# Algolzw/image-restoration-sde

Measured on AMD Instinct MI355X. Metric: restored images/sec at 256x256, 100-step IR-SDE reverse sampler, higher is better.
Workload: dtype f32; 1 GPU; IR-SDE deraining ConditionalUNet nf=64 depth=4, reverse_sde, batch=16/GPU 256x256, T=100 (BASELINE.json configs[1]); compute_dtype=fp32, global_batch=16

## Files before the change

### image_restoration_sde_amd/csrc/engine_api.hip

```cpp
#include "engine.h"
#include <cmath>
#include "../../include/irsde_hip_debug.h"

using namespace irsde;

namespace irsde {
namespace {

thread_local std::string g_last_error;

hipEvent_t get_event(irsde_engine* e, size_t i) {
    while (e->ev_pool.size() <= i) {
        hipEvent_t ev;
        IRSDE_HIP_CHECK(hipEventCreate(&ev));
        e->ev_pool.push_back(ev);
    }
    return e->ev_pool[i];
}

void run_net(Plan* pl, hipStream_t s) {
    for (auto& op : pl->net_ops) op.fn(s);
}

UpdateParams make_update(irsde_engine* e, Plan* pl) {
    UpdateParams u{};
    u.x = pl->xin; u.mu = pl->cin; u.pred = pl->pred;
    const int64_t ps = pl->pred_stride;
    u.sb = (int64_t)pl->Hp * pl->Wp * ps; u.sc = 1; u.sy = (int64_t)pl->Wp * ps; u.sx = ps;
    u.st = pl->own_step ? pl->own_step : e->step; u.ctl = e->ctl;
    u.B = pl->B; u.C = e->cfg.in_nc; u.H = pl->H; u.W = pl->W;
    u.batch0 = pl->b0;
    return u;
}

void one_step(irsde_engine* e, Plan* pl, hipStream_t s) {
    launch_step_begin(e->step, e->film_table, e->film_row, e->film_cur, e->coef_table, s);
    run_net(pl, s);
    launch_sde_update(make_update(e, pl), s);
}

void ensure_sub_streams(irsde_engine* e, int n) {
    if (!e->ev_fork) IRSDE_HIP_CHECK(hipEventCreateWithFlags(&e->ev_fork, hipEventDisableTiming));
    for (int i = 0; i + 1 < n; ++i) {
        if (!e->sub_stream[i]) IRSDE_HIP_CHECK(hipStreamCreateWithFlags(&e->sub_stream[i], hipStreamNonBlocking));
        if (!e->ev_join[i]) IRSDE_HIP_CHECK(hipEventCreateWithFlags(&e->ev_join[i], hipEventDisableTiming));
    }
}
void one_step_part(irsde_engine* e, Plan* pl, hipStream_t s) {
    launch_step_begin(pl->own_step, e->film_table, e->film_row, pl->own_film, e->coef_table, s);
    run_net(pl, s);
    launch_sde_update(make_update(e, pl), s);
}

struct VariantScope {
    explicit VariantScope(int v) { conv_set_variant(v); }
    ~VariantScope() { conv_set_variant(0); }
};

bool code_in(const std::initializer_list<int>& codes, int c) { return std::find(codes.begin(), codes.end(), c) != codes.end(); }
bool debug_conv_code_known(int c) {
    return code_in({0, 1, 2, 3, 4, 5, 12, 13, 22, 23, 33, 34, 35, 36, 37, 42, 43, 44, 45, 46, 47, 55, 56, 62, 63, 204, 260, 261, 262, 263}, c) ||
           code_in({100, 103, 105, 106, 107, 150, 160, 161, 162, 163, 165, 166, 167, 170, 171, 172, 173}, c);
}
bool bench_conv_variant_known(int v) {
    return code_in({0, 3, 5, 6, 7, 50, 60, 61, 62, 63, 64, 65, 66, 67, 70, 71, 72, 73}, v) ||
           code_in({80, 81, 82, 412, 413, 421, 422, 423, 430, 431, 432, 434, 435, 460, 461, 462, 465, 467, 468, 469, 480, 481, 482}, v) ||
           code_in({2001, 2002, 2004, 4650, 4651, 4652, 4653}, v) ||
           (v >= 83 && v <= 82 + 255) ||
           (v >= 472 && v <= 476);
}

void apply_fp16_flag(irsde_engine* e) {
    if (!(e->cfg.flags & IRSDE_FLAG_FP16)) return;
    if (e->cfg.flags & IRSDE_FLAG_BF16_ACT) {
        delete e;
        throw HipError("IRSDE_FLAG_FP16 keeps fp32 activation storage: it cannot be combined with IRSDE_FLAG_BF16_ACT");
    }
    e->cfg.flags |= IRSDE_FLAG_BF16;
}

int guard(const std::function<void()>& f) {
    try {
        f();
        return IRSDE_OK;
    } catch (const HipError& ex) {
        g_last_error = ex.what();
        const std::string m = ex.what();
        if (m.find("weight") != std::string::npos) return IRSDE_ERR_WEIGHT;
        if (m.find(" failed: ") != std::string::npos) return IRSDE_ERR_HIP;
        return IRSDE_ERR_INVALID;
    } catch (const std::exception& ex) {
        g_last_error = ex.what();
        return IRSDE_ERR_INVALID;
    }
}

}
}

extern "C" {

const char* irsde_last_error(void) { return g_last_error.c_str(); }
int irsde_version(void) { return 107; }

int irsde_create(const irsde_config* cfg, irsde_engine** out) {
    return guard([&] {
        if (!cfg || !out) throw HipError("null argument");
        if (cfg->nf % 32 || cfg->nf < 32) throw HipError("nf must be a positive multiple of 32");
        if (cfg->depth < 1 || cfg->depth > 6) throw HipError("depth out of range");
        if (cfg->in_nc < 1 || cfg->in_nc > 4 || cfg->out_nc < 1 || cfg->out_nc > 4)
            throw HipError("in_nc/out_nc must be in 1..4");
        if (cfg->in_nc != cfg->out_nc) throw HipError("sampler needs in_nc == out_nc");
        if ((cfg->nf << cfg->depth) > 2048) throw HipError("nf * 2^depth must be <= 2048");
        if (cfg->flags & IRSDE_FLAG_NAF_STEREO) throw HipError("IRSDE_FLAG_NAF_STEREO: the stereo network is a ConditionalNAFNet (irsde_create_nafnet)");
        if (cfg->flags & IRSDE_FLAG_NAF_UNCOND) throw HipError("IRSDE_FLAG_NAF_UNCOND: irsde_create_nafnet only (the unconditional UNet is IRSDE_FLAG_UNCOND_FULLATTN)");
        auto* e = new irsde_engine();
        e->cfg = *cfg;
        if (cfg->flags & IRSDE_FLAG_BF16_ACT) {
            if (cfg->flags & (IRSDE_FLAG_UNCOND_FULLATTN | IRSDE_FLAG_NAIVE_CONV)) {
                delete e;
// ... 456 lines not shown
int irsde_debug_scam(const float* x, int B, int H, int W, int C, const float* norm_l_g, const float* norm_r_g, const float* l_proj1_w,
                     const float* l_proj1_b, const float* r_proj1_w, const float* r_proj1_b, const float* l_proj2_w, const float* l_proj2_b,
                     const float* r_proj2_w, const float* r_proj2_b, const float* beta, const float* gamma, float* out, void* stream) {
    return guard([&] {
        if (!x || !out || !norm_l_g || !norm_r_g || !l_proj1_w || !l_proj1_b || !r_proj1_w || !r_proj1_b || !l_proj2_w || !l_proj2_b || !r_proj2_w ||
            !r_proj2_b || !beta || !gamma)
            throw HipError("null argument");
        if (B < 1) throw HipError("debug_scam: bad shape");
        scam_check_shape(H, W, C);
        hipStream_t s = reinterpret_cast<hipStream_t>(stream);
        conv_global_init();
        const int Hs = H / 4, Ws = W / 4;
        std::vector<float> wl, bl, wr, br;
        scam_pack_proj(l_proj1_w, l_proj1_b, l_proj2_w, l_proj2_b, C, wl, bl);
        scam_pack_proj(r_proj1_w, r_proj1_b, r_proj2_w, r_proj2_b, C, wr, br);
        std::vector<float*> bufs;
        auto up = [&](const float* h, size_t n) {
            float* d = nullptr;
            IRSDE_HIP_CHECK(hipMalloc(&d, std::max<size_t>(n, 16) * 4));
            bufs.push_back(d);
            if (h) IRSDE_HIP_CHECK(hipMemcpy(d, h, n * 4, hipMemcpyHostToDevice));
            return d;
        };
        try {
            float *dgl = up(norm_l_g, C), *dgr = up(norm_r_g, C), *dbe = up(beta, C), *dga = up(gamma, C);
            float *dwl = up(wl.data(), wl.size()), *dbl = up(bl.data(), bl.size()), *dwr = up(wr.data(), wr.size()), *dbr = up(br.data(), br.size());
            const size_t vsz = (size_t)B * Hs * Ws * 2 * C;
            float *xs2 = up(nullptr, 2 * vsz), *qv = up(nullptr, 2 * vsz), *F = up(nullptr, vsz), *dz = up(nullptr, 256);
            IRSDE_HIP_CHECK(hipMemset(dz, 0, 1024));
            launch_scam_prologue(x, dgl, dgr, xs2, B, H, W, C, s);
            for (int v = 0; v < 2; ++v) {
                ConvParams p;
                p.in0 = xs2 + v * vsz; p.C0 = 2 * C; p.pix0 = 2 * C;
                p.Hin = Hs; p.Win = Ws;
                p.w = v ? dwr : dwl; p.Cout = 2 * C; p.KH = p.KW = 1; p.stride = 1;
                p.B = B; p.Ho = Hs; p.Wo = Ws;
                p.out = qv + v * vsz; p.out_stride = 2 * C;
                p.bias = v ? dbr : dbl;
                p.zeros = dz;
                launch_conv(p, s);
            }
            launch_scam_core(qv, F, B, H, W, C, s);
            launch_scam_epilogue(x, F, dbe, dga, out, B, H, W, C, s);
            IRSDE_HIP_CHECK(hipStreamSynchronize(s));
        } catch (...) {
            (void)hipStreamSynchronize(s);
            for (float* p : bufs) (void)hipFree(p);
            throw;
        }
        for (float* p : bufs) (void)hipFree(p);
    });
}

int irsde_debug_conv(const float* in0, int C0, const float* in1, int C1, int B, int Hin, int Win, int in_shift,
                     const float* w_oihw, int Cout, int KH, int KW, int stride, int pad, const float* bias,
                     const float* film, int film_bstride, int silu, const float* res, float* out, int naive,
                     int splits, void* stream) {
    return guard([&] {
        if (!in0 || !w_oihw || !out) throw HipError("null argument");
        if (!debug_conv_code_known(naive)) throw HipError("debug_conv: unknown selector code " + std::to_string(naive));
        hipStream_t s = reinterpret_cast<hipStream_t>(stream);
        conv_global_init();
        const int Cin = C0 + C1;
        std::vector<float> pk((size_t)Cout * KH * KW * Cin);
        for (int o = 0; o < Cout; ++o)
            for (int i = 0; i < Cin; ++i)
                for (int ky = 0; ky < KH; ++ky)
                    for (int kx = 0; kx < KW; ++kx)
                        pk[(((size_t)o * KH + ky) * KW + kx) * Cin + i] = w_oihw[(((size_t)o * Cin + i) * KH + ky) * KW + kx];
        float *dw = nullptr, *db = nullptr, *dp = nullptr;
        IRSDE_HIP_CHECK(hipMalloc(&dw, pk.size() * 4));
        IRSDE_HIP_CHECK(hipMemcpy(dw, pk.data(), pk.size() * 4, hipMemcpyHostToDevice));
        if (bias) {
            IRSDE_HIP_CHECK(hipMalloc(&db, Cout * 4));
            IRSDE_HIP_CHECK(hipMemcpy(db, bias, Cout * 4, hipMemcpyHostToDevice));
        }
        ConvParams p;
        p.in0 = in0; p.C0 = C0; p.pix0 = C0; p.in1 = in1; p.C1 = C1; p.pix1 = C1;
        p.Hin = Hin; p.Win = Win; p.in_shift = in_shift;
        p.w = dw; p.Cout = Cout; p.KH = KH; p.KW = KW; p.stride = stride; p.pad_y = pad; p.pad_x = pad;
        p.B = B;
        p.Ho = ((Hin << in_shift) + 2 * pad - KH) / stride + 1;
        p.Wo = ((Win << in_shift) + 2 * pad - KW) / stride + 1;
        p.out = out; p.out_stride = Cout; p.bias = db; p.film = film; p.film_bstride = film_bstride; p.silu = silu;
        p.res = res; p.res_stride = Cout;
        float* dz = nullptr;
        IRSDE_HIP_CHECK(hipMalloc(&dz, 1024));
        IRSDE_HIP_CHECK(hipMemset(dz, 0, 1024));
        p.zeros = dz;
        const int wino_tile = (naive == 2 || naive == 12 || naive == 22) ? 2 : (naive == 3 || naive == 13 || naive == 23) ? 4 : 0;
        if (splits > 1 && naive != 1 && !wino_tile) {
            p.splits = splits;
            IRSDE_HIP_CHECK(hipMalloc(&dp, (size_t)splits * B * p.Ho * p.Wo * Cout * 4));
            p.partial = dp;
        }
        if (naive == 44 || naive == 45) {
            const bool f16 = naive == 44;
            if (!wino_shape_ok(p, 4) || Cin % 32) throw HipError("debug_conv: shape not eligible for the pair GEMM");
            std::vector<float> U((size_t)36 * Cout * Cin);
            wino_transform_weights(pk.data(), Cout, Cin, U.data(), 4);
            float mx = 0.f;
            for (float v : U) mx = std::max(mx, std::fabs(v));
            const float us = f16 && mx > 0.f ? std::exp2(std::floor(std::log2(512.0f / mx))) : 1.f;
            const long long T = (long long)B * (p.Ho / 4) * (p.Wo / 4);
            float *dU = nullptr, *dM = nullptr;
            unsigned short *dUp = nullptr, *dVp = nullptr;
            IRSDE_HIP_CHECK(hipMalloc(&dU, U.size() * 4));
            IRSDE_HIP_CHECK(hipMemcpy(dU, U.data(), U.size() * 4, hipMemcpyHostToDevice));
            IRSDE_HIP_CHECK(hipMalloc(&dUp, U.size() * 4));
            IRSDE_HIP_CHECK(hipMalloc(&dVp, (size_t)36 * T * Cin * 4));
            IRSDE_HIP_CHECK(hipMalloc(&dM, (size_t)36 * T * Cout * 4));
            launch_split_pairs(dU, dUp, (size_t)36 * Cout, Cin, s, f16, us);
            const WinoSplitPlan sp = make_wino_pairs(p, dUp, dVp, dM, f16, us);
            launch_wino_input(sp.in, s);
            launch_gemm_split_pairs(sp.gemm, 36, s, 0, f16);
            launch_wino_output(sp.out, s);
            IRSDE_HIP_CHECK(hipStreamSynchronize(s));
            (void)hipFree(dU); (void)hipFree(dUp); (void)hipFree(dVp); (void)hipFree(dM);
        } else if (naive == 42 || naive == 43) {
            const int npl = naive - 40;
            if (!wino_shape_ok(p, 4)) throw HipError("debug_conv: shape not eligible for Winograd");
            std::vector<float> U((size_t)36 * Cout * Cin);
            wino_transform_weights(pk.data(), Cout, Cin, U.data(), 4);
            const long long T = (long long)B * (p.Ho / 4) * (p.Wo / 4);
            float *dU = nullptr, *dM = nullptr;
            unsigned short *dUs = nullptr, *dVs = nullptr;
            IRSDE_HIP_CHECK(hipMalloc(&dU, U.size() * 4));
            IRSDE_HIP_CHECK(hipMemcpy(dU, U.data(), U.size() * 4, hipMemcpyHostToDevice));
            IRSDE_HIP_CHECK(hipMalloc(&dUs, U.size() * 2 * npl));
            IRSDE_HIP_CHECK(hipMalloc(&dVs, (size_t)36 * T * Cin * 2 * npl));
            IRSDE_HIP_CHECK(hipMalloc(&dM, (size_t)36 * T * Cout * 4));
            launch_split_planes(dU, dUs, U.size(), U.size(), npl, s);
            const WinoSplitPlan sp = make_wino_split(p, dUs, dVs, dM, npl);
            launch_wino_input(sp.in, s);
            launch_gemm_split(sp.gemm, npl, 36, s);
            launch_wino_output(sp.out, s);
            IRSDE_HIP_CHECK(hipStreamSynchronize(s));
            (void)hipFree(dU); (void)hipFree(dUs); (void)hipFree(dVs); (void)hipFree(dM);
// ... 409 lines not shown
                IRSDE_HIP_CHECK(hipMalloc(&dM, (size_t)36 * T * Cout * 4));
                wp = make_wino(p, dU, dV, dM, 4);
                if (variant == 421) launch_wino_input(wp.in, s);
            }
            if (split_v) {
                if (!wino_shape_ok(p, 4)) throw HipError("bench_conv: shape not eligible for Winograd F(4x4,3x3)");
                const int npl = variant % 10;
                const long long T = (long long)B * (p.Ho / 4) * (p.Wo / 4);
                const size_t nu = (size_t)36 * Cout * Cin;
                IRSDE_HIP_CHECK(hipMalloc(&dUs, nu * 2 * npl));
                IRSDE_HIP_CHECK(hipMalloc(&dVs, (size_t)36 * T * Cin * 2 * npl));
                IRSDE_HIP_CHECK(hipMalloc(&dM, (size_t)36 * T * Cout * 4));
                launch_split_planes(dU, dUs, nu, nu, npl, s);
                sp = make_wino_split(p, dUs, dVs, dM, npl);
                launch_wino_input(sp.in, s);
            }
        }
        if (variant == 82) {
            IRSDE_HIP_CHECK(hipMalloc(&dU, (size_t)36 * nw / 9 * 4));
            launch_fill_random(dU, (size_t)36 * nw / 9, 5, 1.0f / sqrtf((float)(9 * Cin)), s);
            const int nb = wino_fused_num_blocks(p);
            unsigned long long* dd = nullptr;
            IRSDE_HIP_CHECK(hipMalloc(&dd, (size_t)nb * 128 * 8));
            launch_wino_fused(p, dU, s);
            IRSDE_HIP_CHECK(hipMemsetAsync(dd, 0, (size_t)nb * 128 * 8, s));
            launch_wino_fused(p, dU, s, dd);
            IRSDE_HIP_CHECK(hipStreamSynchronize(s));
            std::vector<unsigned long long> hd((size_t)nb * 128);
            IRSDE_HIP_CHECK(hipMemcpy(hd.data(), dd, hd.size() * 8, hipMemcpyDeviceToHost));
            double ph[2][4] = {{0, 0, 0, 0}, {0, 0, 0, 0}};
            unsigned long long rt_min = ~0ull, rt_max = 0;
            for (int bi = 0; bi < nb; ++bi)
                for (int w = 0; w < 8; ++w) {
                    const unsigned long long* t = &hd[((size_t)bi * 8 + w) * 16];
                    for (int k = 0; k < 4; ++k) ph[w >= 4][k] += (double)(t[k + 1] - t[k]) / ((double)nb * 4);
                    rt_min = std::min(rt_min, t[7]);
                    rt_max = std::max(rt_max, t[7]);
                }
            printf("wino_fused timeline B=%d %dx%d Cin=%d Cout=%d: %d blocks, block starts span %.1f us\n", B, p.Ho, p.Wo, Cin, Cout, nb,
                   (double)(rt_max - rt_min) / 100.0);
            printf("  MFMA waves     (shader cycles): start->V[0] ready %.0f | K loop %.0f | acc->LDS+barrier %.0f | epilogue %.0f\n", ph[0][0],
                   ph[0][1], ph[0][2], ph[0][3]);
            printf("  producer waves (shader cycles): start->chunk 0 done %.0f | K loop rest %.0f | wait MFMA+acc %.0f | epilogue %.0f\n",
                   ph[1][0], ph[1][1], ph[1][2], ph[1][3]);
            fflush(stdout);
            (void)hipFree(dd);
            (void)hipFree(dU);
            dU = nullptr;
            *ms_out = 0.0;
            (void)hipFree(din); (void)hipFree(dw); (void)hipFree(dout); (void)hipFree(dres); (void)hipFree(dfilm);
            (void)hipStreamDestroy(s);
            return;
        }
        if (variant == 465 || (variant >= 4650 && variant <= 4653)) {
            if (!wino_fused64t_eligible(p)) throw HipError("bench_conv: shape not eligible for the two-tile-group fused Winograd kernel");
            const int nbp = 256;
            unsigned long long* dd = nullptr;
            IRSDE_HIP_CHECK(hipMalloc(&dd, (size_t)nbp * 64 * 8));
            launch_wino_fused64t(p, dU, s, 0);
            IRSDE_HIP_CHECK(hipMemsetAsync(dd, 0, (size_t)nbp * 64 * 8, s));
            wino_fused64t_set_debug(dd);
            launch_wino_fused64t(p, dU, s, variant == 465 ? 5 : 12 + (variant - 4650));
            IRSDE_HIP_CHECK(hipStreamSynchronize(s));
            wino_fused64t_set_debug(nullptr);
            std::vector<unsigned long long> hd((size_t)nbp * 64);
            IRSDE_HIP_CHECK(hipMemcpy(hd.data(), dd, hd.size() * 8, hipMemcpyDeviceToHost));
            double a5[8] = {0, 0, 0, 0, 0, 0, 0, 0};
            int nwv = 0;
            for (int bi = 0; bi < nbp; ++bi)
                for (int w = 0; w < 8; ++w) {
                    const unsigned long long* t = &hd[((size_t)bi * 8 + w) * 8];
                    if (!t[3]) continue;
                    for (int k = 0; k < 8; ++k) a5[k] += (double)t[k];
                    nwv++;
                }
            const int nst = Cin / 16;
            const double items = a5[4] / std::max(nwv, 1), chunks = items * nst;
            printf("wino4_fused64t stamps B=%d %dx%d Cin=%d Cout=%d: %.1f items x %d chunks of 16 channels per block; shader cycles per wave (mean over %d waves)\n", B, p.Ho, p.Wo, Cin,
                   Cout, items, nst, nwv);
            printf("  kernel %.0f = K loops incl. transform slices %.0f (%.0f per chunk; MFMA floor per SIMD 9216) + chunk barrier waits %.0f (%.0f per chunk) + epilogue, exchange, first-chunk transform %.0f (%.0f per item)\n",
                   a5[3] / nwv, a5[0] / nwv, a5[0] / nwv / chunks, a5[1] / nwv, a5[1] / nwv / chunks, (a5[2] + a5[5] + a5[6] + a5[7]) / nwv, (a5[2] + a5[5] + a5[6] + a5[7]) / nwv / items);
            printf("  per item: first stage + exchange writes + ring %.0f | exchange barriers + reads %.0f | second stage, stores, gathers %.0f | zero, first-chunk transform, barrier %.0f\n",
                   a5[5] / nwv / items, a5[6] / nwv / items, a5[7] / nwv / items, a5[2] / nwv / items);
            fflush(stdout);
            (void)hipFree(dd);
            (void)hipFree(dU);
            dU = nullptr;
            *ms_out = 0.0;
            (void)hipFree(din); (void)hipFree(dw); (void)hipFree(dout); (void)hipFree(dres); (void)hipFree(dfilm);
            (void)hipStreamDestroy(s);
            return;
        }
        if (variant == 435 || (variant >= 2001 && variant <= 2004)) {
            const int stamp_variant = variant == 2001 ? 28 : variant == 2002 ? 29 : 25;
            const int nbp = 256;
            unsigned long long* dd = nullptr;
            IRSDE_HIP_CHECK(hipMalloc(&dd, (size_t)nbp * 64 * 8));
            launch_wino_fused64(p, dU, s, 20);
            IRSDE_HIP_CHECK(hipMemsetAsync(dd, 0, (size_t)nbp * 64 * 8, s));
            wino_fused64_set_debug(dd);
            launch_wino_fused64(p, dU, s, stamp_variant);
            IRSDE_HIP_CHECK(hipStreamSynchronize(s));
            wino_fused64_set_debug(nullptr);
            std::vector<unsigned long long> hd((size_t)nbp * 64);
            IRSDE_HIP_CHECK(hipMemcpy(hd.data(), dd, hd.size() * 8, hipMemcpyDeviceToHost));
            double acc[2][5] = {{0, 0, 0, 0, 0}, {0, 0, 0, 0, 0}};
            int nw[2] = {0, 0};
// ... 265 lines not shown
```

### image_restoration_sde_amd/csrc/wino_fused_t.hip

```cpp
#include "common.h"
#include "wino_fused_shared.h"
#include <mutex>

namespace irsde {

namespace {

constexpr int WT_NT = 512;
constexpr int WT_KC = 16;
constexpr int WT_PS = 256;
constexpr int WT_ZS = 2 * WT_PS;
constexpr int WT_VBUF = 36 * WT_ZS;
constexpr int WT_XCH_BYTES = 8 * 12 * 64 * 16;
constexpr int WT_RES_BYTES = 8 * 8 * 1024;
constexpr int WT_LDS_BYTES = 160 * 1024;
static_assert(WT_XCH_BYTES + WT_RES_BYTES <= WT_LDS_BYTES && 2 * WT_VBUF * 4 <= WT_LDS_BYTES, "LDS budget");
constexpr unsigned WT_ROW_OOB = 0x80000000u;
constexpr unsigned WT_COL_OOB = 0x40000000u;

__device__ __forceinline__ void swap32x6(float& a0, float& b0, float& a1, float& b1, float& a2, float& b2, float& a3, float& b3, float& a4, float& b4,
                                         float& a5, float& b5) {
    asm volatile(
        "s_nop 1\n\tv_permlane32_swap_b32 %0, %1\n\tv_permlane32_swap_b32 %2, %3\n\tv_permlane32_swap_b32 %4, %5\n\t"
        "v_permlane32_swap_b32 %6, %7\n\tv_permlane32_swap_b32 %8, %9\n\tv_permlane32_swap_b32 %10, %11"
        : "+v"(a0), "+v"(b0), "+v"(a1), "+v"(b1), "+v"(a2), "+v"(b2), "+v"(a3), "+v"(b3), "+v"(a4), "+v"(b4), "+v"(a5), "+v"(b5));
}

template <int H>
__device__ __forceinline__ void wt_stage1(const floatx4 (&acc)[18][2], floatx4 (&keep)[12], float* xs) {
#pragma unroll
    for (int tg = 0; tg < 2; ++tg) {
        floatx4 u[4][3];
#pragma unroll
        for (int sc = 0; sc < 3; ++sc) {
            const floatx4 m0 = acc[sc][tg], m1 = acc[3 + sc][tg], m2 = acc[6 + sc][tg], m3 = acc[9 + sc][tg], m4 = acc[12 + sc][tg], m5 = acc[15 + sc][tg];
            const floatx4 s12 = m1 + m2, d12 = m1 - m2, s34 = m3 + m4, d34 = m3 - m4;
            u[0][sc] = m0 + s12 + s34;
            u[1][sc] = d12 + 2.0f * d34;
            u[2][sc] = s12 + 4.0f * s34;
            u[3][sc] = d12 + 8.0f * d34 + m5;
        }
#pragma unroll
        for (int i = 0; i < 4; ++i) {
            const floatx4 t0 = H == 0 ? u[i][0] : u[i][0] + u[i][1];
            const floatx4 t1 = H == 0 ? u[i][1] + u[i][2] : u[i][0] - u[i][1];
            const floatx4 t2 = H == 0 ? u[i][1] - u[i][2] : u[i][2];
            if (tg == H) {
                keep[3 * i] = t0; keep[3 * i + 1] = t1; keep[3 * i + 2] = t2;
            } else {
                *reinterpret_cast<floatx4*>(xs + (3 * i) * 256) = t0;
                *reinterpret_cast<floatx4*>(xs + (3 * i + 1) * 256) = t1;
                *reinterpret_cast<floatx4*>(xs + (3 * i + 2) * 256) = t2;
            }
        }
    }
}

template <int H, int HALF, bool RES, bool SILU>
__device__ __forceinline__ void wt_finish_rows(const ConvParams& p, const floatx4 (&keep)[12], const floatx4 (&recv)[12], const floatx4 (&rv)[2][4],
                                               const unsigned lane_off_out, const __amdgpu_buffer_rsrc_t rs_out, const floatx4 bias, const floatx4 fsc,
                                               const floatx4 fsh) {
    constexpr int AUX = 2;
    const int orow = p.Wo * p.out_stride * 4, opix = p.out_stride * 4;
#pragma unroll
    for (int ii = 0; ii < 2; ++ii) {
        const int i = 2 * HALF + ii;
        const floatx4 u0 = H == 0 ? keep[3 * i] : recv[3 * i], s12 = H == 0 ? keep[3 * i + 1] : recv[3 * i + 1], d12 = H == 0 ? keep[3 * i + 2] : recv[3 * i + 2];
        const floatx4 s34 = H == 0 ? recv[3 * i] : keep[3 * i], d34 = H == 0 ? recv[3 * i + 1] : keep[3 * i + 1], u5 = H == 0 ? recv[3 * i + 2] : keep[3 * i + 2];
        floatx4 y[4];
        y[0] = u0 + s12 + s34;
        y[1] = d12 + 2.0f * d34;
        y[2] = s12 + 4.0f * s34;
        y[3] = d12 + 8.0f * d34 + u5;
#pragma unroll
        for (int j = 0; j < 4; ++j) {
            floatx4 v = (y[j] + bias) * fsc + fsh;
            if constexpr (SILU) {
                v.x = silu_w(v.x); v.y = silu_w(v.y); v.z = silu_w(v.z); v.w = silu_w(v.w);
            }
            if constexpr (RES) v = v + rv[ii][j];
            __builtin_amdgcn_raw_buffer_store_b128(__builtin_bit_cast(__attribute__((__vector_size__(4 * sizeof(unsigned)))) unsigned, v), rs_out,
                                                   (int)(lane_off_out + (unsigned)(i * orow + j * opix)), 0, AUX);
        }
    }
}

constexpr int WT_NR = 6;

template <bool NOWT, bool NOPATCH, int EPI, bool STAMP = false, int DBG = 0>
__global__ __launch_bounds__(WT_NT, 2) void wino4_fused64t_kernel(const ConvParams p, const float* __restrict__ Uf, const int GX, const int GY, const int NB,
                                                                   const unsigned in0_bytes, const unsigned in1_bytes, const unsigned uf_bytes,
                                                                   const unsigned out_bytes, const unsigned res_bytes, const int xcd_nb, const int total,
                                                                   unsigned long long* __restrict__ dbg) {
    static_assert(18 % WT_NR == 0, "the ring must divide the 18 weight units of a chunk");
    constexpr bool RES = (EPI & 2) != 0, SILU = (EPI & 1) != 0;
    unsigned long long st_a = 0, st_b = 0, st_c = 0, st_n = 0, st_t0 = 0, st_t = 0, st_e1 = 0, st_e2 = 0, st_e3 = 0;
    if constexpr (STAMP) st_t0 = st_t = __builtin_amdgcn_s_memtime();
#define WT_STAMP(ACC)                                                     \
    if constexpr (STAMP) {                                                \
        const unsigned long long now_ = __builtin_amdgcn_s_memtime();     \
        ACC += now_ - st_t;                                               \
        st_t = now_;                                                      \
    }
    extern __shared__ __attribute__((aligned(16))) float smem[];
    const int tid = threadIdx.x;
    const int lane = tid & 63;
    const int wave = __builtin_amdgcn_readfirstlane(tid >> 6);
    const int cb = wave & 3, h = wave >> 2;
    const int TH = p.Ho >> 2, TW = p.Wo >> 2;
    const int Ctot = p.C0 + p.C1;
    const int nch = Ctot / WT_KC;
    const int nblocks = gridDim.x;
    const int l15 = lane & 15, g = lane >> 4;
    const __amdgpu_buffer_rsrc_t rsrc_u = __builtin_amdgcn_make_buffer_rsrc(const_cast<float*>(Uf), 0, NOWT ? 0u : uf_bytes, 0x00020000);
    const __amdgpu_buffer_rsrc_t rs_out = __builtin_amdgcn_make_buffer_rsrc(p.out, 0, out_bytes, 0x00020000);
    const __amdgpu_buffer_rsrc_t rs_res = __builtin_amdgcn_make_buffer_rsrc(const_cast<float*>(p.res ? p.res : p.out), 0, p.res ? res_bytes : 0u, 0x00020000);
    floatx4 acc[18][2];
    const floatx4 kZero4 = {0.f, 0.f, 0.f, 0.f};
    const int uv_lane = lane * 16;
    const int zstride = NB * nch * 4096;
    int v = blockIdx.x;
    W6Item it = w6_item(v, total, NB, GX, GY, xcd_nb);
    int ubase = it.nblk * nch * 4096 + cb * 1024 + 3 * h * zstride;
    auto unit_rel = [&](const int zl) { return ((zl / 3) * 6 + zl % 3) * zstride; };
    floatx4 ring[WT_NR];
    const int v_lane = g * 64 + (((l15 ^ (2 * g)) & 15) * 4);
    const __amdgpu_buffer_rsrc_t rsrc0 = __builtin_amdgcn_make_buffer_rsrc(const_cast<float*>(p.in0), 0, NOPATCH ? 0u : in0_bytes, 0x00020000);
    const __amdgpu_buffer_rsrc_t rsrc1 =
        __builtin_amdgcn_make_buffer_rsrc(const_cast<float*>(p.in1 ? p.in1 : p.in0), 0, (p.in1 && !NOPATCH) ? in1_bytes : 0u, 0x00020000);
    const int hh = lane >> 5, tl = (lane >> 3) & 3, cp = lane & 7;
    const int ptile = 4 * (wave & 3) + tl, ptg = wave >> 2;
    const int kg = cp >> 1;
    const int vw_base = hh * (18 * WT_ZS) + ptg * WT_PS + kg * 64 + (((ptile ^ (2 * kg)) & 15) * 4) + 2 * (cp & 1);
    const int Hv = p.Hin << p.in_shift, Wv = p.Win << p.in_shift;
    floatx2 raw[18];
    unsigned rowoff[6], coloff[3];
#pragma unroll
// ... 92 lines not shown
                    if (u < 3) { WT_GATHER_ROW(2 * u) WT_GATHER_ROW(2 * u + 1) }                                             \
                    if (u == 2) { WT_ADVANCE() WT_SETUP() }                                                                  \
                }                                                                                                            \
                if constexpr (!(DBG & 1)) { if (u >= TC && u < TC + 3) WT_COLPASS(u - TC) }                                  \
                if constexpr (!(DBG & 4)) { if (u == TC + 3) WT_SWAPS() }                                                    \
                if constexpr (!(DBG & 2)) { if (u >= TC + 4 && u < TC + 7) WT_ROWPASS_WRITE(u - TC - 4, wbuf) }              \
                if constexpr (GA && !(DBG & 8)) {                                                                            \
                    if constexpr (FIRST) {                                                                                   \
                        if (u >= 16) { WT_GATHER_ROW(3 * (u - 16)) WT_GATHER_ROW(3 * (u - 16) + 1) WT_GATHER_ROW(3 * (u - 16) + 2) } \
                    } else {                                                                                                 \
                        if (u >= 13 && u < 16) { WT_GATHER_ROW(2 * (u - 13)) WT_GATHER_ROW(2 * (u - 13) + 1) }               \
                    }                                                                                                        \
                }                                                                                                            \
                __builtin_amdgcn_sched_barrier(0);                                                                           \
            }                                                                                                                \
            if (!(LAST) || u + WT_NR < 18) {    \
                const int K = u + WT_NR;                                                                                     \
                const int off = K < 18 ? cur_off + unit_rel(K) : cur_off + 4096 + unit_rel(K - 18);                          \
                ring[u % WT_NR] = __builtin_bit_cast(floatx4, __builtin_amdgcn_raw_buffer_load_b128(rsrc_u, uv_lane, off, 0)); \
            }                                                                                                                \
            __builtin_amdgcn_sched_barrier(0);                                                                               \
        }                                                                                                                    \
        if constexpr (GA) WT_ADVANCE()                                                                                       \
        WT_STAMP(st_a)                                                                                                       \
        __syncthreads();                                                                                                     \
        WT_STAMP(st_b)                                                                                                       \
    }

    WT_SETUP()
#pragma unroll
    for (int i = 0; i < 6; ++i) WT_GATHER_ROW(i)
    WT_ADVANCE()
#pragma unroll
    for (int i = 0; i < WT_NR; ++i)
        ring[i] = __builtin_bit_cast(floatx4, __builtin_amdgcn_raw_buffer_load_b128(rsrc_u, uv_lane, ubase + unit_rel(i), 0));
#pragma unroll
    for (int j = 0; j < 3; ++j) WT_COLPASS(j)
    WT_SWAPS()
#pragma unroll
    for (int r = 0; r < 3; ++r) WT_ROWPASS_WRITE(r, 0)
    WT_SETUP()
    __syncthreads();
    WT_STAMP(st_c)
    while (v < total) {
        const int nv = v + nblocks;
        nit = w6_item(nv < total ? nv : v, total, NB, GX, GY, xcd_nb);
        const int nubase = nit.nblk * nch * 4096 + cb * 1024 + 3 * h * zstride;
        WT_CHUNK(0, true, true, false, true)
        for (int c = 1; c < nch - 2; ++c) WT_CHUNK(c, true, true, false, false)
        WT_CHUNK(nch - 2, true, false, false, false)
        WT_CHUNK(nch - 1, false, false, true, false)
        {
            const int n = it.nblk * 64 + cb * 16 + 4 * g;
            const int tyy = it.gy * 4 + (l15 >> 2), txx = it.gx * 8 + h * 4 + (l15 & 3);
            const bool ok = tyy < TH && txx < TW;
            const unsigned pix = (unsigned)((it.b * p.Ho + 4 * tyy) * p.Wo + 4 * txx);
            unsigned off_out = ok ? (pix * (unsigned)p.out_stride + (unsigned)n) * 4u : WF_OOB;
            unsigned off_res = ok ? (pix * (unsigned)p.res_stride + (unsigned)n) * 4u : WF_OOB;
            if constexpr ((DBG & 128) != 0) {
                const int tx4 = it.gx * 8 + h * 4 + cb;
                const unsigned pixc = (unsigned)((it.b * p.Ho + 4 * tyy) * p.Wo + 4 * tx4);
                const unsigned nn = (unsigned)(it.nblk * 64 + ((l15 & 3) * 4 + g) * 4);
                off_out = (tyy < TH && tx4 < TW) ? (pixc * (unsigned)p.out_stride + nn) * 4u : WF_OOB;
                off_res = (tyy < TH && tx4 < TW) ? (pixc * (unsigned)p.res_stride + nn) * 4u : WF_OOB;
            }
            constexpr int AUX = 2;
            const int rrow = p.Wo * p.res_stride * 4, rpix = p.res_stride * 4;
            floatx4 rv0[2][4], rv1[2][4];
            char* const rslot = reinterpret_cast<char*>(smem) + WT_XCH_BYTES + wave * 8192;
            if constexpr (RES) {
#pragma unroll
                for (int i = 0; i < 2; ++i)
#pragma unroll
                    for (int j = 0; j < 4; ++j)
                        __builtin_amdgcn_raw_ptr_buffer_load_lds(rs_res, (__attribute__((address_space(3))) void*)(rslot + (i * 4 + j) * 1024), 16, (int)off_res, i * rrow + j * rpix, 0, AUX);
                __builtin_amdgcn_sched_barrier(0);
            }
            floatx4 keep[12];
            float* xs = smem + (wave * 12 * 64 + lane) * 4;
            if (h == 0) wt_stage1<0>(acc, keep, xs); else wt_stage1<1>(acc, keep, xs);
            __builtin_amdgcn_sched_barrier(0);
#pragma unroll
            for (int i = 0; i < WT_NR; ++i)
                ring[i] = __builtin_bit_cast(floatx4, __builtin_amdgcn_raw_buffer_load_b128(rsrc_u, uv_lane, nubase + unit_rel(i), 0));
            floatx4 bias = {0.f, 0.f, 0.f, 0.f}, fsc = {1.f, 1.f, 1.f, 1.f}, fsh = {0.f, 0.f, 0.f, 0.f};
            if (p.bias) bias = *reinterpret_cast<const floatx4*>(p.bias + n);
            if (p.film) {
                const float* f = p.film + (size_t)it.b * p.film_bstride;
                fsc = *reinterpret_cast<const floatx4*>(f + n) + 1.0f;
                fsh = *reinterpret_cast<const floatx4*>(f + p.Cout + n);
            }
            WT_STAMP(st_e1)
            __syncthreads();
            floatx4 recv[12];
            const float* xr = smem + ((wave ^ 4) * 12 * 64 + lane) * 4;
#pragma unroll
            for (int k = 0; k < 12; ++k) recv[k] = *reinterpret_cast<const floatx4*>(xr + k * 256);
            __syncthreads();
            WT_STAMP(st_e2)
            if constexpr (RES) {
                asm volatile("s_waitcnt vmcnt(0)" ::: "memory");
#pragma unroll
                for (int i = 0; i < 2; ++i)
#pragma unroll
                    for (int j = 0; j < 4; ++j) rv0[i][j] = *reinterpret_cast<const floatx4*>(rslot + (i * 4 + j) * 1024 + lane * 16);
                asm volatile("s_waitcnt lgkmcnt(0)" ::: "memory");
#pragma unroll
                for (int i = 0; i < 2; ++i)
#pragma unroll
                    for (int j = 0; j < 4; ++j)
                        __builtin_amdgcn_raw_ptr_buffer_load_lds(rs_res, (__attribute__((address_space(3))) void*)(rslot + (i * 4 + j) * 1024), 16, (int)off_res, (2 + i) * rrow + j * rpix, 0, AUX);
                __builtin_amdgcn_sched_barrier(0);
            }
            WT_SETUP()
#pragma unroll
            for (int i = 0; i < 6; ++i) WT_GATHER_ROW(i)
            WT_ADVANCE()
            __builtin_amdgcn_sched_barrier(0);
            if (h == 0) wt_finish_rows<0, 0, RES, SILU>(p, keep, recv, rv0, off_out, rs_out, bias, fsc, fsh);
            else wt_finish_rows<1, 0, RES, SILU>(p, keep, recv, rv0, off_out, rs_out, bias, fsc, fsh);
            __builtin_amdgcn_sched_barrier(0);
            if constexpr (RES) {
                asm volatile("s_waitcnt vmcnt(26)" ::: "memory");
#pragma unroll
                for (int i = 0; i < 2; ++i)
#pragma unroll
                    for (int j = 0; j < 4; ++j) rv1[i][j] = *reinterpret_cast<const floatx4*>(rslot + (i * 4 + j) * 1024 + lane * 16);
            }
            if (h == 0) wt_finish_rows<0, 1, RES, SILU>(p, keep, recv, rv1, off_out, rs_out, bias, fsc, fsh);
            else wt_finish_rows<1, 1, RES, SILU>(p, keep, recv, rv1, off_out, rs_out, bias, fsc, fsh);
            WT_STAMP(st_e3)
        }
        v = nv; it = nit; ubase = nubase;
        if (v < total) {
#pragma unroll
            for (int j = 0; j < 3; ++j) WT_COLPASS(j)
            WT_SWAPS()
#pragma unroll
            for (int r = 0; r < 3; ++r) WT_ROWPASS_WRITE(r, 0)
            WT_SETUP()
        }
        __syncthreads();
        if constexpr (STAMP) st_n += 1;
        WT_STAMP(st_c)
    }
#undef WT_CHUNK
#undef WT_ROWPASS_WRITE
#undef WT_SWAPS
#undef WT_COLPASS
#undef WT_ADVANCE
#undef WT_GATHER_ROW
#undef WT_SETUP
    if constexpr (STAMP) {
        if (lane == 0 && dbg) {
            unsigned long long* d = dbg + ((size_t)blockIdx.x * 8 + wave) * 8;
            d[0] = st_a; d[1] = st_b; d[2] = st_c; d[3] = __builtin_amdgcn_s_memtime() - st_t0; d[4] = st_n; d[5] = st_e1; d[6] = st_e2; d[7] = st_e3;
        }
    }
#undef WT_STAMP
}

}

long long wino_fused64t_num_items(const ConvParams& p) {
    return (long long)p.B * ((p.Ho / 4 + 3) / 4) * ((p.Wo / 4 + 7) / 8) * (p.Cout / 64);
}

bool wino_fused64t_eligible(const ConvParams& p) {
    if (!wino_fused64_eligible(p)) return false;
    const double lim = 1073741824.0 - 65536.0;
    if (4.0 * p.B * p.Hin * p.Win * (double)p.pix0 >= lim || (p.C1 && 4.0 * p.B * p.Hin * p.Win * (double)p.pix1 >= lim)) return false;
    return true;
}

void wino_fused_t_global_init() {
#define WT_ATTR(...) IRSDE_HIP_CHECK(hipFuncSetAttribute(reinterpret_cast<const void*>(wino4_fused64t_kernel<__VA_ARGS__>), hipFuncAttributeMaxDynamicSharedMemorySize, 160 * 1024))
#define WT_ATTR4(...) WT_ATTR(__VA_ARGS__, 0); WT_ATTR(__VA_ARGS__, 1); WT_ATTR(__VA_ARGS__, 2); WT_ATTR(__VA_ARGS__, 3)
    WT_ATTR4(false, false);
#ifdef IRSDE_PROBES
    WT_ATTR4(true, false);
    WT_ATTR4(false, true);
    WT_ATTR(false, false, 0, true); WT_ATTR(false, false, 1, true);
    WT_ATTR(false, false, 2, true); WT_ATTR(false, false, 3, true);
    WT_ATTR(false, true, 1, true); WT_ATTR(false, true, 3, true);
    WT_ATTR(false, false, 1, false, 7); WT_ATTR(false, false, 3, false, 7);
    WT_ATTR(false, false, 1, false, 15); WT_ATTR(false, false, 3, false, 15);
    WT_ATTR(false, false, 1, false, 8); WT_ATTR(false, false, 3, false, 8);
    WT_ATTR(false, false, 1, true, 128); WT_ATTR(false, false, 3, true, 128);
#endif
#undef WT_ATTR4
#undef WT_ATTR
}

static unsigned long long* g_wt_dbg = nullptr;
void wino_fused64t_set_debug(unsigned long long* buf) { g_wt_dbg = buf; }

void launch_wino_fused64t(const ConvParams& p, const float* Uf, hipStream_t s, int variant) {
    if (!wino_fused64t_eligible(p)) throw HipError("launch_wino_fused64t: layer not eligible");
    if (!Uf) throw HipError("launch_wino_fused64t: fused weights missing");
    const int TH = p.Ho / 4, TW = p.Wo / 4;
    const int GX = (TW + 7) / 8, GY = (TH + 3) / 4, NB = p.Cout / 64;
    const unsigned in0_bytes = (unsigned)((size_t)p.B * p.Hin * p.Win * p.pix0 * 4);
    const unsigned in1_bytes = p.C1 ? (unsigned)((size_t)p.B * p.Hin * p.Win * p.pix1 * 4) : 0u;
    const unsigned uf_bytes = (unsigned)((size_t)36 * p.Cout * (p.C0 + p.C1) * 4);
    const long long G_ = (long long)p.B * GY * GX;
    const int total = (int)(G_ * NB);
    const bool force_xnb = (variant & 64) != 0;
    variant &= 63;
    const bool xnb_legal = NB >= 2 && 8 % NB == 0 && G_ % (8 / NB) == 0;
    const int xcd_nb = (force_xnb ? xnb_legal : (xnb_legal && wino_fused64_xcd_nb(p))) ? 1 : 0;
    const size_t npix_out = (size_t)p.B * p.Ho * p.Wo;
    const size_t ob = npix_out * p.out_stride * 4, rb = p.res ? npix_out * p.res_stride * 4 : 0;
    if (ob >= 0x7fff0000ull || rb >= 0x7fff0000ull) throw HipError("launch_wino_fused64t: output / residual tensor too large for 32-bit buffer offsets");
    const unsigned out_bytes = variant == 13 ? 0u : (unsigned)ob, res_bytes = variant == 14 ? 0u : (unsigned)rb;
    const int ncu = device_cu_count();
    const dim3 pgrid((unsigned)std::min(total, std::max(8, ncu & ~7)));
    const int epi = (p.silu ? 1 : 0) | (p.res ? 2 : 0);
#define WT_LAUNCH(...) hipLaunchKernelGGL((wino4_fused64t_kernel<__VA_ARGS__>), pgrid, dim3(WT_NT), WT_LDS_BYTES, s, p, Uf, GX, GY, NB, in0_bytes, in1_bytes, uf_bytes, out_bytes, res_bytes, xcd_nb, total, g_wt_dbg)
#define WT_LAUNCH_EPI(...)                                  \
    switch (epi) {                                          \
        case 0: WT_LAUNCH(__VA_ARGS__, 0); break;           \
        case 1: WT_LAUNCH(__VA_ARGS__, 1); break;           \
        case 2: WT_LAUNCH(__VA_ARGS__, 2); break;           \
        default: WT_LAUNCH(__VA_ARGS__, 3); break;          \
    }
    switch (variant) {
        case 0: WT_LAUNCH_EPI(false, false) break;
#ifdef IRSDE_PROBES
        case 1: WT_LAUNCH_EPI(true, false) break;
        case 2: WT_LAUNCH_EPI(false, true) break;
        case 12:
            if (epi != 1 && epi != 3) throw HipError("launch_wino_fused64t: measurement twins exist for epilogues 1 / 3");
            if (epi == 1) WT_LAUNCH(false, true, 1, true); else WT_LAUNCH(false, true, 3, true);
            break;
        case 15:
            if (epi != 1 && epi != 3) throw HipError("launch_wino_fused64t: measurement twins exist for epilogues 1 / 3");
            if (epi == 1) WT_LAUNCH(false, false, 1, true, 128); else WT_LAUNCH(false, false, 3, true, 128);
            break;
        case 5: case 13: case 14:
            switch (epi) {
                case 0: WT_LAUNCH(false, false, 0, true); break;
                case 1: WT_LAUNCH(false, false, 1, true); break;
                case 2: WT_LAUNCH(false, false, 2, true); break;
                default: WT_LAUNCH(false, false, 3, true); break;
            }
            break;
        case 6: case 7: case 8:
            if (epi != 1 && epi != 3) throw HipError("launch_wino_fused64t: measurement twins exist for epilogues 1 / 3");
            if (variant == 6) { if (epi == 1) WT_LAUNCH(false, false, 1, false, 7); else WT_LAUNCH(false, false, 3, false, 7); }
            if (variant == 7) { if (epi == 1) WT_LAUNCH(false, false, 1, false, 15); else WT_LAUNCH(false, false, 3, false, 15); }
            if (variant == 8) { if (epi == 1) WT_LAUNCH(false, false, 1, false, 8); else WT_LAUNCH(false, false, 3, false, 8); }
            break;
#endif
        default: throw HipError("launch_wino_fused64t: bad variant (the measurement twins need a make PROBES=1 build)");
    }
#undef WT_LAUNCH_EPI
#undef WT_LAUNCH
    IRSDE_HIP_CHECK(hipGetLastError());
}

}
```

Measured before the change: 4.261 images/s.

## Stage Winograd epilogue outputs through LDS for coalesced full-line stores

The fused Winograd 4x4 kernel's epilogue now writes the finished output tiles (with bias, FiLM, SiLU and residual) into swizzled LDS staging buffers. It then reads them back so each lane stores contiguous 16-byte lines to global memory, instead of storing scattered pixels straight from registers. Residual rows are loaded into the staging slots and added in place. The next chunk's ring loads are moved after the bias and FiLM reads. This is meant to improve global store coalescing, at the cost of extra LDS traffic and additional block barriers. A debug entry point with custom output strides is also added, and the DBG-128 probe variant is removed.

```diff
diff --git a/image_restoration_sde_amd/csrc/engine_api.hip b/image_restoration_sde_amd/csrc/engine_api.hip
--- a/image_restoration_sde_amd/csrc/engine_api.hip
+++ b/image_restoration_sde_amd/csrc/engine_api.hip
@@ -65,7 +65,7 @@
 bool bench_conv_variant_known(int v) {
     return code_in({0, 3, 5, 6, 7, 50, 60, 61, 62, 63, 64, 65, 66, 67, 70, 71, 72, 73}, v) ||
            code_in({80, 81, 82, 412, 413, 421, 422, 423, 430, 431, 432, 434, 435, 460, 461, 462, 465, 467, 468, 469, 480, 481, 482}, v) ||
-           code_in({2001, 2002, 2004, 4650, 4651, 4652, 4653}, v) ||
+           code_in({2001, 2002, 2004, 4650, 4651, 4652}, v) ||
            (v >= 83 && v <= 82 + 255) ||
            (v >= 472 && v <= 476);
 }
@@ -628,6 +628,25 @@
     });
 }
 
+static thread_local int g_debug_out_stride = 0, g_debug_res_stride = 0;
+
+int irsde_debug_conv_slot(const float* in0, int C0, const float* in1, int C1, int B, int Hin, int Win, int in_shift,
+                          const float* w_oihw, int Cout, int KH, int KW, int stride, int pad, const float* bias,
+                          const float* film, int film_bstride, int silu, const float* res, int res_stride, float* out, int out_stride,
+                          int naive, void* stream) {
+    const int rc = guard([&] {
+        if (!code_in({34, 36, 55, 62, 63}, naive)) throw HipError("debug_conv_slot: selector " + std::to_string(naive) + " is not a fused Winograd f32 kernel (34, 36, 55, 62, 63)");
+        if (out_stride < Cout || out_stride % 4 || (res && (res_stride < Cout || res_stride % 4))) throw HipError("debug_conv_slot: pixel strides must be multiples of 4 floats and at least Cout");
+        if ((reinterpret_cast<uintptr_t>(out) | reinterpret_cast<uintptr_t>(res)) & 15) throw HipError("debug_conv_slot: slots must start on 16-byte boundaries");
+    });
+    if (rc != IRSDE_OK) return rc;
+    struct Scope {
+        Scope(int o, int r) { g_debug_out_stride = o; g_debug_res_stride = r; }
+        ~Scope() { g_debug_out_stride = g_debug_res_stride = 0; }
+    } scope(out_stride, res ? res_stride : 0);
+    return irsde_debug_conv(in0, C0, in1, C1, B, Hin, Win, in_shift, w_oihw, Cout, KH, KW, stride, pad, bias, film, film_bstride, silu, res, out, naive, 1, stream);
+}
+
 int irsde_debug_conv(const float* in0, int C0, const float* in1, int C1, int B, int Hin, int Win, int in_shift,
                      const float* w_oihw, int Cout, int KH, int KW, int stride, int pad, const float* bias,
                      const float* film, int film_bstride, int silu, const float* res, float* out, int naive,
@@ -658,8 +677,8 @@
         p.B = B;
         p.Ho = ((Hin << in_shift) + 2 * pad - KH) / stride + 1;
         p.Wo = ((Win << in_shift) + 2 * pad - KW) / stride + 1;
-        p.out = out; p.out_stride = Cout; p.bias = db; p.film = film; p.film_bstride = film_bstride; p.silu = silu;
-        p.res = res; p.res_stride = Cout;
+        p.out = out; p.out_stride = g_debug_out_stride ? g_debug_out_stride : Cout; p.bias = db; p.film = film; p.film_bstride = film_bstride; p.silu = silu;
+        p.res = res; p.res_stride = g_debug_res_stride ? g_debug_res_stride : Cout;
         float* dz = nullptr;
         IRSDE_HIP_CHECK(hipMalloc(&dz, 1024));
         IRSDE_HIP_CHECK(hipMemset(dz, 0, 1024));
@@ -1175,7 +1194,7 @@
             (void)hipStreamDestroy(s);
             return;
         }
-        if (variant == 465 || (variant >= 4650 && variant <= 4653)) {
+        if (variant == 465 || (variant >= 4650 && variant <= 4652)) {
             if (!wino_fused64t_eligible(p)) throw HipError("bench_conv: shape not eligible for the two-tile-group fused Winograd kernel");
             const int nbp = 256;
             unsigned long long* dd = nullptr;
diff --git a/image_restoration_sde_amd/csrc/wino_fused_t.hip b/image_restoration_sde_amd/csrc/wino_fused_t.hip
--- a/image_restoration_sde_amd/csrc/wino_fused_t.hip
+++ b/image_restoration_sde_amd/csrc/wino_fused_t.hip
@@ -11,10 +11,14 @@
 constexpr int WT_PS = 256;
 constexpr int WT_ZS = 2 * WT_PS;
 constexpr int WT_VBUF = 36 * WT_ZS;
+constexpr int WT_STG_BYTES = 8 * 8 * 1024;
 constexpr int WT_XCH_BYTES = 8 * 12 * 64 * 16;
-constexpr int WT_RES_BYTES = 8 * 8 * 1024;
+constexpr int WT_STA_OFF = 0;
+constexpr int WT_XCH_OFF = WT_STG_BYTES;
+constexpr int WT_STB_OFF = 96 * 1024;
 constexpr int WT_LDS_BYTES = 160 * 1024;
-static_assert(WT_XCH_BYTES + WT_RES_BYTES <= WT_LDS_BYTES && 2 * WT_VBUF * 4 <= WT_LDS_BYTES, "LDS budget");
+static_assert(WT_XCH_OFF + WT_XCH_BYTES <= WT_LDS_BYTES && WT_STB_OFF + WT_STG_BYTES <= WT_LDS_BYTES && 2 * WT_VBUF * 4 <= WT_LDS_BYTES, "LDS budget");
+static_assert(WT_STA_OFF + WT_STG_BYTES <= WT_XCH_OFF && WT_STB_OFF >= WT_VBUF * 4, "staging A must not touch the exchange, staging B must not touch V[0]");
 constexpr unsigned WT_ROW_OOB = 0x80000000u;
 constexpr unsigned WT_COL_OOB = 0x40000000u;
 
@@ -57,11 +61,8 @@
 }
 
 template <int H, int HALF, bool RES, bool SILU>
-__device__ __forceinline__ void wt_finish_rows(const ConvParams& p, const floatx4 (&keep)[12], const floatx4 (&recv)[12], const floatx4 (&rv)[2][4],
-                                               const unsigned lane_off_out, const __amdgpu_buffer_rsrc_t rs_out, const floatx4 bias, const floatx4 fsc,
+__device__ __forceinline__ void wt_finish_rows(const floatx4 (&keep)[12], const floatx4 (&recv)[12], char* const st, const floatx4 bias, const floatx4 fsc,
                                                const floatx4 fsh) {
-    constexpr int AUX = 2;
-    const int orow = p.Wo * p.out_stride * 4, opix = p.out_stride * 4;
 #pragma unroll
     for (int ii = 0; ii < 2; ++ii) {
         const int i = 2 * HALF + ii;
@@ -78,11 +79,24 @@
             if constexpr (SILU) {
                 v.x = silu_w(v.x); v.y = silu_w(v.y); v.z = silu_w(v.z); v.w = silu_w(v.w);
             }
-            if constexpr (RES) v = v + rv[ii][j];
-            __builtin_amdgcn_raw_buffer_store_b128(__builtin_bit_cast(__attribute__((__vector_size__(4 * sizeof(unsigned)))) unsigned, v), rs_out,
-                                                   (int)(lane_off_out + (unsigned)(i * orow + j * opix)), 0, AUX);
-        }
-    }
+            floatx4* const slot = reinterpret_cast<floatx4*>(st + (ii * 4 + j) * 1024);
+            if constexpr (RES) v = v + *slot;
+            *slot = v;
+        }
+    }
+}
+
+template <int HALF>
+__device__ __forceinline__ void wt_store_lines(const ConvParams& p, const char* const rows, const unsigned lane_off_out, const __amdgpu_buffer_rsrc_t rs_out) {
+    constexpr int AUX = 2;
+    const int orow = p.Wo * p.out_stride * 4, opix = p.out_stride * 4;
+    floatx4 t[8];
+#pragma unroll
+    for (int k = 0; k < 8; ++k) t[k] = *reinterpret_cast<const floatx4*>(rows + k * 1024);
+#pragma unroll
+    for (int k = 0; k < 8; ++k)
+        __builtin_amdgcn_raw_buffer_store_b128(__builtin_bit_cast(__attribute__((__vector_size__(4 * sizeof(unsigned)))) unsigned, t[k]), rs_out,
+                                               (int)(lane_off_out + (unsigned)((2 * HALF + (k >> 2)) * orow + (k & 3) * opix)), 0, AUX);
 }
 
 constexpr int WT_NR = 6;
@@ -281,37 +295,31 @@
         WT_CHUNK(nch - 1, false, false, true, false)
         {
             const int n = it.nblk * 64 + cb * 16 + 4 * g;
-            const int tyy = it.gy * 4 + (l15 >> 2), txx = it.gx * 8 + h * 4 + (l15 & 3);
+            const int lt = lane >> 4;
+            const int tyy = it.gy * 4 + cb, txx = it.gx * 8 + h * 4 + lt;
             const bool ok = tyy < TH && txx < TW;
             const unsigned pix = (unsigned)((it.b * p.Ho + 4 * tyy) * p.Wo + 4 * txx);
-            unsigned off_out = ok ? (pix * (unsigned)p.out_stride + (unsigned)n) * 4u : WF_OOB;
-            unsigned off_res = ok ? (pix * (unsigned)p.res_stride + (unsigned)n) * 4u : WF_OOB;
-            if constexpr ((DBG & 128) != 0) {
-                const int tx4 = it.gx * 8 + h * 4 + cb;
-                const unsigned pixc = (unsigned)((it.b * p.Ho + 4 * tyy) * p.Wo + 4 * tx4);
-                const unsigned nn = (unsigned)(it.nblk * 64 + ((l15 & 3) * 4 + g) * 4);
-                off_out = (tyy < TH && tx4 < TW) ? (pixc * (unsigned)p.out_stride + nn) * 4u : WF_OOB;
-                off_res = (tyy < TH && tx4 < TW) ? (pixc * (unsigned)p.res_stride + nn) * 4u : WF_OOB;
-            }
+            const unsigned nl = (unsigned)(it.nblk * 64 + 4 * ((lane & 15) ^ (cb * 4 + lt)));
+            const unsigned off_out = ok ? (pix * (unsigned)p.out_stride + nl) * 4u : WF_OOB;
+            const unsigned off_res = ok ? (pix * (unsigned)p.res_stride + nl) * 4u : WF_OOB;
             constexpr int AUX = 2;
             const int rrow = p.Wo * p.res_stride * 4, rpix = p.res_stride * 4;
-            floatx4 rv0[2][4], rv1[2][4];
-            char* const rslot = reinterpret_cast<char*>(smem) + WT_XCH_BYTES + wave * 8192;
+            char* const sm = reinterpret_cast<char*>(smem);
+            char* const line_a = sm + WT_STA_OFF + wave * 8192;
+            char* const line_b = sm + WT_STB_OFF + wave * 8192;
+            const int mine = (h * 4 + (l15 >> 2)) * 8192 + ((l15 & 3) * 16 + ((cb * 4 + g) ^ l15)) * 16;
             if constexpr (RES) {
 #pragma unroll
                 for (int i = 0; i < 2; ++i)
 #pragma unroll
                     for (int j = 0; j < 4; ++j)
-                        __builtin_amdgcn_raw_ptr_buffer_load_lds(rs_res, (__attribute__((address_space(3))) void*)(rslot + (i * 4 + j) * 1024), 16, (int)off_res, i * rrow + j * rpix, 0, AUX);
+                        __builtin_amdgcn_raw_ptr_buffer_load_lds(rs_res, (__attribute__((address_space(3))) void*)(line_a + (i * 4 + j) * 1024), 16, (int)off_res, i * rrow + j * rpix, 0, AUX);
                 __builtin_amdgcn_sched_barrier(0);
             }
             floatx4 keep[12];
-            float* xs = smem + (wave * 12 * 64 + lane) * 4;
+            float* xs = smem + WT_XCH_OFF / 4 + (wave * 12 * 64 + lane) * 4;
             if (h == 0) wt_stage1<0>(acc, keep, xs); else wt_stage1<1>(acc, keep, xs);
             __builtin_amdgcn_sched_barrier(0);
-#pragma unroll
-            for (int i = 0; i < WT_NR; ++i)
-                ring[i] = __builtin_bit_cast(floatx4, __builtin_amdgcn_raw_buffer_load_b128(rsrc_u, uv_lane, nubase + unit_rel(i), 0));
             floatx4 bias = {0.f, 0.f, 0.f, 0.f}, fsc = {1.f, 1.f, 1.f, 1.f}, fsh = {0.f, 0.f, 0.f, 0.f};
             if (p.bias) bias = *reinterpret_cast<const floatx4*>(p.bias + n);
             if (p.film) {
@@ -319,26 +327,27 @@
                 fsc = *reinterpret_cast<const floatx4*>(f + n) + 1.0f;
                 fsh = *reinterpret_cast<const floatx4*>(f + p.Cout + n);
             }
+            __builtin_amdgcn_sched_barrier(0);
+#pragma unroll
+            for (int i = 0; i < WT_NR; ++i)
+                ring[i] = __builtin_bit_cast(floatx4, __builtin_amdgcn_raw_buffer_load_b128(rsrc_u, uv_lane, nubase + unit_rel(i), 0));
+            if constexpr (RES) asm volatile("s_waitcnt vmcnt(%0)" ::"n"(WT_NR) : "memory");
             WT_STAMP(st_e1)
             __syncthreads();
             floatx4 recv[12];
-            const float* xr = smem + ((wave ^ 4) * 12 * 64 + lane) * 4;
+            const float* xr = smem + WT_XCH_OFF / 4 + ((wave ^ 4) * 12 * 64 + lane) * 4;
 #pragma unroll
             for (int k = 0; k < 12; ++k) recv[k] = *reinterpret_cast<const floatx4*>(xr + k * 256);
+            if (h == 0) wt_finish_rows<0, 0, RES, SILU>(keep, recv, sm + WT_STA_OFF + mine, bias, fsc, fsh);
+            else wt_finish_rows<1, 0, RES, SILU>(keep, recv, sm + WT_STA_OFF + mine, bias, fsc, fsh);
             __syncthreads();
             WT_STAMP(st_e2)
             if constexpr (RES) {
-                asm volatile("s_waitcnt vmcnt(0)" ::: "memory");
 #pragma unroll
                 for (int i = 0; i < 2; ++i)
 #pragma unroll
-                    for (int j = 0; j < 4; ++j) rv0[i][j] = *reinterpret_cast<const floatx4*>(rslot + (i * 4 + j) * 1024 + lane * 16);
-                asm volatile("s_waitcnt lgkmcnt(0)" ::: "memory");
-#pragma unroll
-                for (int i = 0; i < 2; ++i)
-#pragma unroll
                     for (int j = 0; j < 4; ++j)
-                        __builtin_amdgcn_raw_ptr_buffer_load_lds(rs_res, (__attribute__((address_space(3))) void*)(rslot + (i * 4 + j) * 1024), 16, (int)off_res, (2 + i) * rrow + j * rpix, 0, AUX);
+                        __builtin_amdgcn_raw_ptr_buffer_load_lds(rs_res, (__attribute__((address_space(3))) void*)(line_b + (i * 4 + j) * 1024), 16, (int)off_res, (2 + i) * rrow + j * rpix, 0, AUX);
                 __builtin_amdgcn_sched_barrier(0);
             }
             WT_SETUP()
@@ -346,18 +355,20 @@
             for (int i = 0; i < 6; ++i) WT_GATHER_ROW(i)
             WT_ADVANCE()
             __builtin_amdgcn_sched_barrier(0);
-            if (h == 0) wt_finish_rows<0, 0, RES, SILU>(p, keep, recv, rv0, off_out, rs_out, bias, fsc, fsh);
-            else wt_finish_rows<1, 0, RES, SILU>(p, keep, recv, rv0, off_out, rs_out, bias, fsc, fsh);
+            if constexpr (!RES) {
+                if (h == 0) wt_finish_rows<0, 1, RES, SILU>(keep, recv, sm + WT_STB_OFF + mine, bias, fsc, fsh);
+                else wt_finish_rows<1, 1, RES, SILU>(keep, recv, sm + WT_STB_OFF + mine, bias, fsc, fsh);
+            }
+            wt_store_lines<0>(p, line_a + lane * 16, off_out, rs_out);
             __builtin_amdgcn_sched_barrier(0);
             if constexpr (RES) {
                 asm volatile("s_waitcnt vmcnt(26)" ::: "memory");
-#pragma unroll
-                for (int i = 0; i < 2; ++i)
-#pragma unroll
-                    for (int j = 0; j < 4; ++j) rv1[i][j] = *reinterpret_cast<const floatx4*>(rslot + (i * 4 + j) * 1024 + lane * 16);
-            }
-            if (h == 0) wt_finish_rows<0, 1, RES, SILU>(p, keep, recv, rv1, off_out, rs_out, bias, fsc, fsh);
-            else wt_finish_rows<1, 1, RES, SILU>(p, keep, recv, rv1, off_out, rs_out, bias, fsc, fsh);
+                __syncthreads();
+                if (h == 0) wt_finish_rows<0, 1, RES, SILU>(keep, recv, sm + WT_STB_OFF + mine, bias, fsc, fsh);
+                else wt_finish_rows<1, 1, RES, SILU>(keep, recv, sm + WT_STB_OFF + mine, bias, fsc, fsh);
+            }
+            __syncthreads();
+            wt_store_lines<1>(p, line_b + lane * 16, off_out, rs_out);
             WT_STAMP(st_e3)
         }
         v = nv; it = nit; ubase = nubase;
@@ -415,7 +426,6 @@
     WT_ATTR(false, false, 1, false, 7); WT_ATTR(false, false, 3, false, 7);
     WT_ATTR(false, false, 1, false, 15); WT_ATTR(false, false, 3, false, 15);
     WT_ATTR(false, false, 1, false, 8); WT_ATTR(false, false, 3, false, 8);
-    WT_ATTR(false, false, 1, true, 128); WT_ATTR(false, false, 3, true, 128);
 #endif
 #undef WT_ATTR4
 #undef WT_ATTR
@@ -462,10 +472,6 @@
             if (epi != 1 && epi != 3) throw HipError("launch_wino_fused64t: measurement twins exist for epilogues 1 / 3");
             if (epi == 1) WT_LAUNCH(false, true, 1, true); else WT_LAUNCH(false, true, 3, true);
             break;
-        case 15:
-            if (epi != 1 && epi != 3) throw HipError("launch_wino_fused64t: measurement twins exist for epilogues 1 / 3");
-            if (epi == 1) WT_LAUNCH(false, false, 1, true, 128); else WT_LAUNCH(false, false, 3, true, 128);
-            break;
         case 5: case 13: case 14:
             switch (epi) {
                 case 0: WT_LAUNCH(false, false, 0, true); break;
```

New measurement: 4.300 images/s (median of 6 runs). About the same (+0.9%).
